# JacobMackay/beifong

Hardware: AMD Instinct MI355X
Metric: Mrays/s (closest + any-hit BVH queries), Bus.obj-class radar scene (higher is better)
Workload: dtype f32

## Files before the change

beifong_amd/csrc/bf_api.cpp:

```cpp
#include <algorithm>
#include <cmath>
#include <cstdarg>
#include <cstdio>
#include <cstring>
#include <limits>
#include <new>
#include <string>

#include <dlfcn.h>
#if defined(__has_include) && __has_include(<rccl/rccl.h>)
#include <rccl/rccl.h>
#else
extern "C" {
typedef struct ncclComm *ncclComm_t;
typedef enum { ncclSuccess = 0 } ncclResult_t;
typedef enum { ncclFloat = 7 } ncclDataType_t;
typedef enum { ncclSum = 0 } ncclRedOp_t;
ncclResult_t ncclCommInitAll(ncclComm_t *comm, int ndev, const int *devlist);
ncclResult_t ncclCommDestroy(ncclComm_t comm);
ncclResult_t ncclAllReduce(const void *sendbuff, void *recvbuff, size_t count, ncclDataType_t datatype, ncclRedOp_t op, ncclComm_t comm,
                           hipStream_t stream);
ncclResult_t ncclGroupStart(void);
ncclResult_t ncclGroupEnd(void);
const char *ncclGetErrorString(ncclResult_t result);
}
#endif

#include <map>
#include <mutex>

#include "bf_scene.h"


static thread_local std::string g_err;

bf_status fail(bf_status st, const char *fmt, ...) {
    char buf[512];
    va_list ap;
    va_start(ap, fmt);
    vsnprintf(buf, sizeof(buf), fmt, ap);
    va_end(ap);
    g_err = buf;
    return st;
}

namespace {
template <typename T> bf_status upload(const std::vector<T> &v, const T **out, std::vector<void *> &owned, uint64_t &bytes) {
    *out = nullptr;
    if (v.empty()) return BF_OK;
    void *p = nullptr;
    HIP_TRY(hipMalloc(&p, v.size() * sizeof(T)));
    owned.push_back(p);
    HIP_TRY(hipMemcpy(p, v.data(), v.size() * sizeof(T), hipMemcpyHostToDevice));
    bytes += v.size() * sizeof(T);
    *out = reinterpret_cast<const T *>(p);
    return BF_OK;
}
}

static bf_tunables read_tunables() {
    bf_tunables t;
    auto num = [](const char *name, long long dflt) -> long long {
        const char *e = getenv(name);
        return e ? strtoll(e, nullptr, 10) : dflt;
    };
    t.pool = (uint32_t) std::max<long long>(1024, std::min<long long>(num("BF_WF_POOL", 1ll << 24), 1ll << 26));
    t.tail = num("BF_WF_TAIL", -1);
    t.trace_refill = (uint32_t) num("BF_TRACE_REFILL", bfd::kTraceRefill);
    t.trace_stragglers = (uint32_t) num("BF_TRACE_STRAGGLERS", bfd::kTraceStragglers);
    t.shade_chain = (uint32_t) std::max<long long>(1, num("BF_SHADE_CHAIN", bfd::kShadeChain));
    t.row_jobs = (uint32_t) num("BF_TAIL_ROWJOBS", bfd::kTailRowJobs);
    t.shade_waves = (int) std::max<long long>(1, std::min<long long>(4, num("BF_SHADE_WAVES", 3)));
    {
        const long long w = num("BF_TRACE_WAVES", 5);
        t.trace_waves = w < 5 ? 4 : (w > 5 ? 6 : 5);
    }
    t.tail_waves = num("BF_TAIL_WAVES", 3) == 2 ? 2 : 3;
    t.tail_spread = (unsigned) std::max<long long>(1, num("BF_TAIL_SPREAD", 1));
    t.tail_blocks = (unsigned) std::max<long long>(0, num("BF_TAIL_BLOCKS", 0));
    t.tail_share = (int) num("BF_TAIL_SHARE", -1);
    t.allow_plan = num("BF_WF_SYNC", 0) == 0;
    t.roll_iters = (uint32_t) std::max<long long>(0, std::min<long long>(32, num("BF_ROLL_ITERS", 0)));
    t.roll_live = (uint32_t) std::max<long long>(0, std::min<long long>(num("BF_ROLL_LIVE", 0), 1ll << 30));
    t.no_wide = getenv("BF_NO_WIDE_BVH") != nullptr;
    t.quant = num("BF_QUANT_BVH", 0) != 0;
    t.wide_rows_log = (int) num("BF_WIDE_ROWS_LOG", -1);
    t.lean = num("BF_LEAN", 1) != 0;
    t.tab_cache = num("BF_TAB_CACHE", 1) != 0;
    t.shade_split = num("BF_SHADE_SPLIT", 0) != 0;
    t.chain_min = (uint32_t) std::max<long long>(0, std::min<long long>(num("BF_CHAIN_MIN", 16), 64));
    t.grid_share = (uint32_t) std::max<long long>(0, std::min<long long>(num("BF_GRID_SHARE", 3), 16));
    t.grid_small = (uint32_t) std::max<long long>(0, std::min<long long>(num("BF_GRID_SMALL", 1ll << 22), 1ll << 30));
    t.roll_join = num("BF_ROLL_JOIN", 1) != 0;
    t.debug_surv_batches = (uint32_t) std::max<long long>(0, std::min<long long>(num("BF_DEBUG_SURV_BATCHES", 0), 1 << 14));
    return t;
}

extern "C" {

int bf_version(void) { return BF_ABI_VERSION; }
uint32_t bf_abi_sizeof(uint32_t which) {
    static const uint32_t sizes[BF_ABI_STRUCTS] = {sizeof(bf_material), sizeof(bf_shape), sizeof(bf_emitter), sizeof(bf_sensor),
                                                   sizeof(bf_scene_desc), sizeof(bf_launch), sizeof(bf_path_record), sizeof(bf_stats),
                                                   sizeof(bf_scene_info), sizeof(bf_batch)};
    return which < BF_ABI_STRUCTS ? sizes[which] : 0u;
}
uint64_t bf_abi_fingerprint(void) { return BF_ABI_FINGERPRINT; }
const char *bf_last_error(void) { return g_err.c_str(); }

int bf_device_count(void) {
    int n = 0;
    if (hipGetDeviceCount(&n) != hipSuccess) return 0;
    return n;
}

bf_status bf_set_device(int device) {
    HIP_TRY(hipSetDevice(device));
    return BF_OK;
}

static uint32_t film_pixels(const bf_launch *lp) {
    return (lp->spp && lp->film_width && lp->film_height) ? lp->film_width * lp->film_height : 1u;
}

uint32_t bf_launch_channels(const bf_launch *lp) {
    if (!lp) return 0;
    if (lp->flags & BF_FLAG_MOMENT) {
        switch (lp->mode) {
            case BF_MODE_PATH: return 11 * film_pixels(lp);
            case BF_MODE_RANGE: return (11 + 2 * lp->bins) * film_pixels(lp);
            case BF_MODE_TIME: return (11 + 6 * lp->bins) * film_pixels(lp);
            case BF_MODE_RECEIVE_RAW: return (4 + lp->phase_bins) * lp->bins * lp->bins_y;
            case BF_MODE_RECEIVE_IQ: return 5 * lp->bins * lp->bins_y;
        }
        return 0;
    }
    switch (lp->mode) {
        case BF_MODE_PATH: return 5 * film_pixels(lp);
        case BF_MODE_RANGE: return (5 + lp->bins) * film_pixels(lp);
        case BF_MODE_TIME: return (5 + 3 * lp->bins) * film_pixels(lp);
        case BF_MODE_RECEIVE_RAW: return (3 + lp->phase_bins) * lp->bins * lp->bins_y;
        case BF_MODE_RECEIVE_IQ: return 3 * lp->bins * lp->bins_y;
    }
    return 0;
}

uint32_t bf_scene_launch_channels(const bf_scene *scene, const bf_launch *lp) {
    const uint32_t n = bf_launch_channels(lp);
    if (scene && lp && (lp->flags & BF_FLAG_AOV) && scene->run.aov.n && lp->mode <= BF_MODE_TIME && !(lp->flags & (BF_FLAG_MOMENT | BF_FLAG_CLASSES))) {
        const uint64_t all = (uint64_t) n + (uint64_t) film_pixels(lp) * (bf_aov_floats(scene->run.aov.n, scene->run.aov.types) + 4u);
        return all > UINT32_MAX ? 0u : (uint32_t) all;
    }
    if (!scene || !lp || !(lp->flags & BF_FLAG_CLASSES)) return n;
    const uint64_t all = (uint64_t) n * std::max(1u, bfd::scene_n_classes(scene->d));
    return all > UINT32_MAX ? 0u : (uint32_t) all;
}

bf_status bf_scene_destroy(bf_scene *s) {
    if (!s) return BF_OK;
    (void) s->run.last.wait();
    if (s->run.roll.open && s->peers_rolling) s->peers_rolling->fetch_sub(1, std::memory_order_relaxed);
    for (void *p : s->owned) (void) hipFree(p);
    for (auto &st : s->stage) {
        if (st.ev) {
            (void) hipEventSynchronize(st.ev);
            (void) hipEventDestroy(st.ev);
        }
        if (st.host) (void) hipHostFree(st.host);
        if (st.dev) (void) hipFree(st.dev);
    }
    delete s;
    return BF_OK;
}

bf_status stage_acquire(const bf_scene *sc, size_t bytes, bf_scene::Stage **out) {
    bf_scene::Stage &st = sc->stage[sc->stage_next];
    sc->stage_next = (sc->stage_next + 1) % bf_scene::kStageSlots;
    if (st.busy) {
        HIP_TRY(hipEventSynchronize(st.ev));
        st.busy = false;
    }
    if (st.cap < bytes) {
        if (st.host) (void) hipHostFree(st.host);
        if (st.dev) (void) hipFree(st.dev);
        st.host = st.dev = nullptr;
        st.cap = 0;
        const size_t cap = std::max<size_t>(4096, (bytes + 4095) & ~size_t(4095));
        HIP_TRY(hipHostMalloc(&st.host, cap));
        HIP_TRY(hipMalloc(&st.dev, cap));
        st.cap = cap;
    }
    if (!st.ev) HIP_TRY(hipEventCreateWithFlags(&st.ev, hipEventDisableTiming));
    *out = &st;
    return BF_OK;
}
bf_status stage_commit(bf_scene::Stage *st, size_t bytes, hipStream_t stream) {
    HIP_TRY(hipMemcpyAsync(st->dev, st->host, bytes, hipMemcpyHostToDevice, stream));
    HIP_TRY(hipEventRecord(st->ev, stream));
    st->busy = true;
    return BF_OK;
}
bf_status stage_release_after(bf_scene::Stage *st, hipStream_t stream) {
    HIP_TRY(hipEventRecord(st->ev, stream));
    st->busy = true;
    return BF_OK;
}

static_assert(bf::kTopNodes == bfd::kTopNodes, "the builder's breadth-first prefix is what wf_trace caches");
static_assert(bfd::CTR_GUARD + 2 == bfd::CTR_COUNT && bfd::CTR_SURV_GUARD + 1 == bfd::CTR_COUNT,
              "the two sticky guard words are the last counters: renders clear the ones before them");

namespace {
struct TriMeta {
    uint32_t prim, shape;
    const float *n0, *n1, *n2;
    const float *uv0, *uv1, *uv2;
};
}

static bf_status gather_triangles(const bf_scene_desc *desc, std::vector<bf::BuildTri> &btris, std::vector<TriMeta> &meta, bool &any_normals,
// ... 903 lines not shown
```

beifong_amd/csrc/bf_render.cpp:

```cpp
#include "bf_scene.h"

#include <algorithm>
#include <cmath>
#include <cstdlib>
#include <cstring>
#include <limits>
#include <vector>

namespace {
struct Kernels {
    decltype(&bfk_launch_render) render;
    decltype(&bfk_wf_shade) shade;
    decltype(&bfk_wf_trace) trace;
    decltype(&bfk_launch_tail) tail;
};
const Kernels kExact = {bfk_launch_render, bfk_wf_shade, bfk_wf_trace, bfk_launch_tail};
const Kernels kFast = {bfk_launch_render_fast, bfk_wf_shade_fast, bfk_wf_trace_fast, bfk_launch_tail_fast};
const Kernels kMoment = {bfk_launch_render_moment, bfk_wf_shade_moment, bfk_wf_trace, bfk_launch_tail_moment};
const Kernels kClass = {bfk_launch_render_class, bfk_wf_shade_class, bfk_wf_trace, bfk_launch_tail_class};
const Kernels kAov = {bfk_launch_render_aov, bfk_wf_shade_aov, bfk_wf_trace, bfk_launch_tail_aov};
const Kernels &kernels_for(uint32_t flags) {
    return (flags & BF_FLAG_FAST) ? kFast : ((flags & BF_FLAG_MOMENT) ? kMoment : ((flags & BF_FLAG_CLASSES) ? kClass : ((flags & BF_FLAG_AOV) ? kAov : kExact)));
}
}

hipError_t RenderState::Feedback::post(const uint32_t *src, uint32_t n_, Owner owner_, hipStream_t stream, const unsigned long long *guards_src) {
    if (pending) return hipSuccess;
    hipError_t e = hipMemcpyAsync(counts, src, n_ * sizeof(uint32_t), hipMemcpyDeviceToHost, stream);
    if (e == hipSuccess && guards_src)
        e = hipMemcpyAsync((void *) guards, guards_src, 2 * sizeof(unsigned long long), hipMemcpyDeviceToHost, stream);
    if (e == hipSuccess) e = hipEventRecord(event, stream);
    if (e != hipSuccess) return e;
    pending = true;
    n = n_;
    owner = owner_;
    return hipSuccess;
}
RenderState::Feedback::Landed RenderState::Feedback::take() {
    const bool ready = pending && hipEventQuery(event) == hipSuccess;
    (void) hipGetLastError();
    if (!ready) return {nullptr, 0, kNone};
    pending = false;
    return {counts, n, owner};
}
uint32_t RenderState::Feedback::first_at_most(const uint32_t *counts, uint32_t n, uint32_t threshold) {
    uint32_t k = 0;
    while (k < n && counts[k] > threshold) ++k;
    return k;
}

RenderState::~RenderState() {
    for (void *p : pool) (void) hipFree(p);
    if (host) (void) hipHostFree(host);
    if (event) (void) hipEventDestroy(event);
    if (fb.counts) (void) hipHostFree(fb.counts);
    if (fb.event) (void) hipEventDestroy(fb.event);
    if (last.done) (void) hipEventDestroy(last.done);
    for (hipEvent_t e : timing) (void) hipEventDestroy(e);
    if (counters) (void) hipFree(counters);
    if (aov.rows) (void) hipFree(aov.rows);
    for (float *q : conv.scratch)
        if (q) (void) hipFree(q);
    if (conv.ws) (void) hipFree(conv.ws);
    if (conv.ring) (void) hipHostFree(conv.ring);
    for (hipEvent_t e : conv.ev)
        if (e) (void) hipEventDestroy(e);
}

extern "C" {

static bf_status wf_ensure(const bf_scene *scene, uint32_t capacity) {
    RenderState &run = scene->run;
    bfd::WF &wf = run.wf;
    if (wf.capacity >= capacity) return BF_OK;
    for (void *p : run.pool) (void) hipFree(p);
    run.pool.clear();
    std::memset(&wf, 0, sizeof(wf));
    run.roll_ring = nullptr;
    run.roll_offsets = nullptr;
    auto alloc = [&](void **p, size_t bytes) -> hipError_t {
        hipError_t e = hipMalloc(p, bytes);
        if (e == hipSuccess) run.pool.push_back(*p);
        return e;
    };
    size_t n = capacity, nb = capacity / 64;
    HIP_TRY(alloc((void **) &wf.recA, n * 64));
    HIP_TRY(alloc((void **) &wf.recB, n * 64));
    HIP_TRY(alloc((void **) &wf.recC, n * 64));
    HIP_TRY(alloc((void **) &run.masks, 8 * nb * sizeof(unsigned long long)));
    HIP_TRY(alloc((void **) &wf.n_live, (bfd::kWfMaxIter + 2) * sizeof(uint32_t)));
    HIP_TRY(alloc((void **) &run.roll_ring, bfd::kRollRing * sizeof(bfd::DRoll)));
    HIP_TRY(alloc((void **) &run.roll_offsets, bfd::kRollRing * sizeof(float4)));
    HIP_TRY(alloc((void **) &wf.surv_cursor, 64));
    wf.counters = run.counters;
    wf.capacity = capacity;
    if (!run.host) HIP_TRY(hipHostMalloc((void **) &run.host, 64));
    if (!run.event) HIP_TRY(hipEventCreateWithFlags(&run.event, hipEventDisableTiming));
    if (!run.fb.counts) HIP_TRY(hipHostMalloc((void **) &run.fb.counts, (bfd::kWfMaxIter + 2) * sizeof(uint32_t)));
    if (!run.fb.event) HIP_TRY(hipEventCreateWithFlags(&run.fb.event, hipEventDisableTiming));
    run.fb.guards = reinterpret_cast<volatile unsigned long long *>(run.host) + 1;
    run.plan.valid = false;
    run.fb.drop();
    return BF_OK;
}

static uint32_t wf_tail_threshold(const bf_scene *scene, uint32_t n_slots) {
    if (scene->tun.tail >= 0) return (uint32_t) scene->tun.tail;
    if (n_slots >= bfd::kTailSmallPool) return 1u << 17;
    return std::max<uint32_t>(1u << 17, std::min<uint32_t>(1u << 19, n_slots / 2));
}

namespace {
struct WfCtx {
    const bf_scene *scene;
    const Kernels *k;
    const bfd::DLaunch *lp;
    float *hist;
    bf_path_record *rec;
    hipStream_t stream;
    bool count_nodes, timed;
    size_t mask_bytes, lds_shade, lds_tail;
    unsigned grid_shade, grid_trace;
    uint32_t tail_max;
    bool alone;
};

static_assert(sizeof(int) * bfd::kStackDepth * bfd::kBlock % 16 == 0, "the stacks keep the histogram 16-byte aligned");
static size_t lds_bytes(const bfd::DLaunch &lp, uint32_t tab_cache, bool stacks) {
    return (stacks ? sizeof(int) * bfd::kStackDepth * bfd::kBlock : 0u) + ((sizeof(float) * lp.lds_floats + 15) & ~size_t(15)) +
           (tab_cache ? bfd::kTabBytes : 0u);
}
static uint32_t lds_hist(uint32_t n_chan, uint32_t flags) {
    return (n_chan <= (uint32_t) bfd::kMaxLdsHist && !(flags & BF_FLAG_GLOBAL_ATOMICS)) ? 1u : 0u;
}
}

static hipError_t wf_tic(const WfCtx &c, int kind) {
    if (!c.timed) return hipSuccess;
    const bf_scene *sc = c.scene;
    while (sc->run.timing.size() < 2 * (sc->run.ev_kind.size() + 1)) {
        hipEvent_t e;
        hipError_t he = hipEventCreate(&e);
        if (he != hipSuccess) return he;
        sc->run.timing.push_back(e);
    }
    sc->run.ev_kind.push_back(kind);
    return hipEventRecord(sc->run.timing[2 * (sc->run.ev_kind.size() - 1)], c.stream);
}
static hipError_t wf_toc(const WfCtx &c) {
    if (!c.timed) return hipSuccess;
    return hipEventRecord(c.scene->run.timing[2 * (c.scene->run.ev_kind.size() - 1) + 1], c.stream);
}
static bf_status wf_collect_timing(const bf_scene *scene, hipStream_t stream) {
    scene->run.ms[0] = scene->run.ms[1] = scene->run.ms[2] = 0.f;
    scene->run.tail_launches = scene->run.shade_launches = 0;
    if (scene->run.ev_kind.empty()) return BF_OK;
    HIP_TRY(hipStreamSynchronize(stream));
    for (size_t k = 0; k < scene->run.ev_kind.size(); ++k) {
        float ms = 0.f;
        HIP_TRY(hipEventElapsedTime(&ms, scene->run.timing[2 * k], scene->run.timing[2 * k + 1]));
        scene->run.ms[scene->run.ev_kind[k]] += ms;
        if (scene->run.ev_kind[k] == 2) ++scene->run.tail_launches;
        if (scene->run.ev_kind[k] == 1) ++scene->run.shade_launches;
    }
    scene->run.ev_kind.clear();
    return BF_OK;
}

static bf_status wf_setup(const bf_scene *scene, const Kernels &k, const bfd::DLaunch &lp, uint64_t pool_paths, float *hist_dev,
                          bf_path_record *records_dev, hipStream_t stream, bool count_nodes, bool timed, WfCtx &c, bool rolling = false) {
    uint64_t want = std::min<uint64_t>(scene->tun.pool, std::max<uint64_t>(pool_paths, 64));
    uint32_t n_main = (uint32_t) ((want + 63) & ~uint64_t(63)), n_surv = 0;
    if (rolling) {
        n_main = (uint32_t) ((std::max<uint64_t>(2 * pool_paths, 128) + 63) & ~uint64_t(63));
        const uint32_t surv_min = (uint32_t) scene->n_cus * 4u * (uint32_t) std::max(2, scene->tun.shade_waves) * 64u;
        n_surv = std::max<uint32_t>(surv_min, std::min<uint32_t>(1u << 21, (n_main / 8 + 63) & ~63u));
        if (scene->tun.debug_surv_batches) n_surv = scene->tun.debug_surv_batches * 64u;
    }
    bf_status st = wf_ensure(scene, n_main + n_surv);
    if (st != BF_OK) return st;
    bfd::WF &wf = scene->run.wf;
    wf.n_main = rolling ? n_main : (uint32_t) ((std::min<uint64_t>(wf.capacity, pool_paths) + 63) & ~uint64_t(63));
    wf.n_surv = n_surv;
    wf.n_slots = wf.n_main + wf.n_surv;
    wf.trace_refill = scene->tun.trace_refill;
    wf.trace_stragglers = scene->tun.trace_stragglers;
    wf.shade_chain = scene->tun.shade_chain;
    wf.row_jobs = scene->tun.row_jobs;
    wf.iq = lp.iq;
    wf.has_render = lp.batch != 0u ? 1u : 0u;
    wf.offsets = lp.batch_offsets;
    wf.has_dop = (lp.doppler || lp.resample) ? 1u : 0u;
    wf.box_slack = lp.box_slack;
    wf.geom_stride = lp.geom_stride;
    const size_t nb = wf.n_slots / 64;
    for (int b = 0; b < 2; ++b) {
        wf.m_alive[b] = scene->run.masks + (4 * b + 0) * nb;
        wf.m_trace[b] = scene->run.masks + (4 * b + 1) * nb;
        wf.m_shadow[b] = scene->run.masks + (4 * b + 2) * nb;
        wf.m_hit[b] = scene->run.masks + (4 * b + 3) * nb;
    }
    c.scene = scene;
    c.k = &k;
    c.lp = &lp;
    c.hist = hist_dev;
    c.rec = records_dev;
    c.stream = stream;
    c.count_nodes = count_nodes;
    c.timed = timed;
    c.mask_bytes = 4 * nb * sizeof(unsigned long long);
    wf.hit_split = scene->tun.shade_split ? 1u : 0u;
    wf.chain_min = scene->tun.chain_min;
    c.lds_shade = lds_bytes(lp, scene->d.tab_cache, false);
    c.lds_tail = lds_bytes(lp, scene->d.tab_cache, true);
    c.alone = false;
    const unsigned batches_per_block = bfd::kBlock / 64;
    const unsigned max_blocks = (unsigned) ((nb + batches_per_block - 1) / batches_per_block);
    c.grid_shade = std::max(1u, std::min((unsigned) scene->n_cus * (unsigned) std::max(2, scene->tun.shade_waves), max_blocks));
    c.grid_trace = std::max(1u, std::min((unsigned) scene->n_cus * (unsigned) scene->tun.trace_waves, max_blocks));
    if (rolling && scene->tun.grid_share > 1u && wf.n_slots < scene->tun.grid_small) {
        const unsigned peers = (unsigned) std::max(1, scene->peers_rolling->load(std::memory_order_relaxed));
        const unsigned share = std::min(peers, (unsigned) scene->tun.grid_share);
        c.grid_shade = std::max(1u, c.grid_shade / share);
        c.grid_trace = std::max(1u, c.grid_trace / share);
    }
    c.tail_max = wf_tail_threshold(scene, rolling ? wf.n_main / 2 : wf.n_slots);
    wf.surv_claims_max = (wf.n_surv / 64u) / std::max(1u, c.grid_shade * batches_per_block);
    if (rolling && scene->tun.debug_surv_batches) {
        const char *e = getenv("BF_DEBUG_SURV_CLAIMS");
        wf.surv_claims_max = e ? (uint32_t) strtoul(e, nullptr, 10) : 1u << 20;
    }
    return BF_OK;
}
static bf_status wf_iteration(const WfCtx &c, uint32_t it, int first) {
    const bf_scene *scene = c.scene;
    const bfd::WF &wf = scene->run.wf;
    const int nxt = (it & 1) ^ 1;
    HIP_TRY(hipMemsetAsync(wf.m_alive[nxt], 0, c.mask_bytes, c.stream));
    if (first != 1) {
        HIP_TRY(wf_tic(c, 1));
        HIP_TRY(c.k->shade(&scene->d, c.lp, &wf, it, first == 2 ? 3 : 0, c.hist, c.rec, c.grid_shade, c.lds_shade, c.stream,
                           scene->tun.shade_waves));
        HIP_TRY(wf_toc(c));
    }
    if (first != 0) {
        HIP_TRY(wf_tic(c, 1));
        HIP_TRY(c.k->shade(&scene->d, c.lp, &wf, it, first, c.hist, c.rec, c.grid_shade, c.lds_shade, c.stream, scene->tun.shade_waves));
        HIP_TRY(wf_toc(c));
    }
    return BF_OK;
}
static bf_status wf_trace_launch(const WfCtx &c, uint32_t it) {
    HIP_TRY(wf_tic(c, 0));
    HIP_TRY(c.k->trace(&c.scene->d, &c.scene->run.wf, it, c.count_nodes ? 1 : 0, c.grid_trace, c.stream, c.scene->tun.trace_waves));
    HIP_TRY(wf_toc(c));
    return BF_OK;
}
static bf_status wf_tail_launch(const WfCtx &c, uint32_t it, uint32_t est_live) {
    const bf_scene *scene = c.scene;
    const bool alone = c.alone;
    uint32_t share = 1;
    if (!alone && scene->tun.tail_share > 1) {
        share = scene->tun.tail_share >= 4 ? 4u : 2u;
        est_live = (uint32_t) std::min<uint64_t>((uint64_t) est_live * share, 1u << 30);
    }
    if (alone) {
        const uint32_t resident = (uint32_t) scene->n_cus * 4u * 3u;
        while (share < 4u && (uint64_t) est_live * (share * 2u) / 64u <= resident) share *= 2u;
        est_live = (uint32_t) std::min<uint64_t>((uint64_t) est_live * share, 1u << 30);
    }
    scene->run.wf.tail_share = share;
    HIP_TRY(wf_tic(c, 2));
    HIP_TRY(c.k->tail(&scene->d, c.lp, &scene->run.wf, it, est_live, c.hist, c.rec, c.count_nodes ? 1 : 0, c.lds_tail, c.stream,
                      scene->tun.tail_waves, scene->tun.tail_spread, scene->tun.tail_blocks));
    HIP_TRY(wf_toc(c));
    return BF_OK;
}
bf_status guard_error(unsigned long long lost, unsigned long long refused) {
    if (lost)
        return fail(BF_ERR_DEVICE, "wf_trace's iteration guard dropped %llu rays in an earlier render of this scene: that render's "
                                   "histogram is wrong (a traversal bug; please report the scene)", lost);
    return fail(BF_ERR_DEVICE, "a launch of a rolling sequence of this scene tried to claim %llu survivor batches beyond the size of "
                               "its survivor area (the claims were refused: no path was lost, but the sizing rule of wf_setup is "
                               "violated; please report the scene and the launch)", refused);
}
bf_status report_guards(const bf_scene *scene, unsigned long long lost, unsigned long long refused, const hipStream_t *async_on) {
    unsigned long long *g = scene->run.counters + bfd::CTR_GUARD;
    if (async_on) HIP_TRY(hipMemsetAsync(g, 0, 2 * sizeof(unsigned long long), *async_on));
    else HIP_TRY(hipMemset(g, 0, 2 * sizeof(unsigned long long)));
    scene->run.fb.drop();
    return guard_error(lost, refused);
}
static bf_status check_film_count(const unsigned long long *c, uint64_t n_paths) {
    if (c[bfd::CTR_FILM] != n_paths)
        return fail(BF_ERR_DEVICE, "%llu of %llu paths were binned: paths were lost or binned twice (a scheduling bug; please report the "
                                   "scene and the launch)", (unsigned long long) c[bfd::CTR_FILM], (unsigned long long) n_paths);
    return BF_OK;
}

static bf_status drive_planned(const WfCtx &c, uint32_t &it, uint32_t n, int first_kind, uint32_t tail_live) {
    bf_status st;
    for (uint32_t j = 0; j < n; ++j, ++it) {
        if ((st = wf_iteration(c, it, j == 0 ? first_kind : 0)) != BF_OK) return st;
        if ((st = wf_trace_launch(c, it)) != BF_OK) return st;
    }
    return wf_tail_launch(c, it, std::max<uint32_t>(tail_live + tail_live / 4, 64u * bfd::kBlock));
}
static bf_status drive_sync(const WfCtx &c, uint32_t &it, uint32_t max_iters, int first_kind, uint32_t *n_live) {
    const RenderState &run = c.scene->run;
    volatile uint32_t *hq = run.host;
    bf_status st;
    for (uint32_t j = 0; j < max_iters; ++j) {
        if ((st = wf_iteration(c, it, j == 0 ? first_kind : 0)) != BF_OK) return st;
        HIP_TRY(hipMemcpyAsync((void *) &hq[0], run.wf.n_live + it, sizeof(uint32_t), hipMemcpyDeviceToHost, c.stream));
        HIP_TRY(hipEventRecord(run.event, c.stream));
        if ((st = wf_trace_launch(c, it)) != BF_OK) return st;
        HIP_TRY(hipEventSynchronize(run.event));
        ++it;
        *n_live = hq[0];
        if (*n_live <= c.tail_max) break;
    }
    return BF_OK;
}

static bf_status aov_attach(const bf_scene *scene, uint64_t slots, bfd::DLaunch &lp);
static bf_status wf_render(const bf_scene *scene, const Kernels &k, const bfd::DLaunch &lp_in, float *hist_dev, bf_path_record *records_dev,
                           hipStream_t stream, bool count_nodes, bool stats, bool aov = false) {
    using Feedback = RenderState::Feedback;
    RenderState &run = scene->run;
    WfCtx c;
    bfd::DLaunch lp = lp_in;
    bf_status st = wf_setup(scene, k, lp, lp.n_paths, hist_dev, records_dev, stream, count_nodes, stats, c);
    if (st != BF_OK) return st;
    bfd::WF &wf = run.wf;
    if (aov && (st = aov_attach(scene, wf.n_slots, lp)) != BF_OK) return st;
    HIP_TRY(hipMemsetAsync(wf.n_live, 0, (bfd::kWfMaxIter + 2) * sizeof(uint32_t), stream));
    run.ev_kind.clear();
    RenderState::Plan &plan = run.plan;
    const Feedback::Landed fb = run.fb.take();
    if (fb.owner == Feedback::kPlan) {
        if (run.fb.guards[0] || run.fb.guards[1]) return report_guards(scene, run.fb.guards[0], run.fb.guards[1], &stream);
        const uint32_t at = Feedback::first_at_most(fb.counts, fb.n, plan.tail_max);
        plan.iters = at < fb.n ? at + 1 : std::min<uint32_t>(fb.n + 2, bfd::kWfMaxIter - 1);
        plan.tail_live = fb.counts[std::min(at, fb.n - 1)];
    }
    uint32_t it = 0;
    if (scene->tun.allow_plan && plan.valid && plan.n_paths == lp.n_paths && plan.mode == lp.mode &&
        plan.max_depth == (uint32_t) lp.max_depth && plan.n_slots == wf.n_slots && plan.tail_max == c.tail_max && plan.iters > 0) {
        if ((st = drive_planned(c, it, plan.iters, 1, plan.tail_live)) != BF_OK) return st;
        HIP_TRY(run.fb.post(wf.n_live, plan.iters, Feedback::kPlan, stream, wf.counters + bfd::CTR_GUARD));
    } else {
        uint32_t n_live = 0;
        if ((st = drive_sync(c, it, bfd::kWfMaxIter, 1, &n_live)) != BF_OK) return st;
        if (n_live > c.tail_max) return fail(BF_ERR_UNSUPPORTED, "path depth exceeded the wavefront iteration limit (%u bounces)", bfd::kWfMaxIter);
        plan = {true, lp.n_paths, lp.mode, (uint32_t) lp.max_depth, wf.n_slots, c.tail_max, it, n_live};
        run.fb.drop();
        if (n_live && (st = wf_tail_launch(c, it, n_live)) != BF_OK) return st;
    }
    run.iters = run.trace_launches = it;
    if (stats) return wf_collect_timing(scene, stream);
    run.ms[0] = run.ms[1] = run.ms[2] = 0.f;
    return BF_OK;
}

static bool roll_same_shape(const bf_launch &a, const bf_launch &b) {
    return a.mode == b.mode && a.color_mode == b.color_mode && a.n_paths == b.n_paths && a.max_depth == b.max_depth &&
           a.rr_depth == b.rr_depth && a.bins == b.bins && a.bins_y == b.bins_y && a.bin_width == b.bin_width &&
           a.time_c == b.time_c && a.flags == b.flags && a.phase_bins == b.phase_bins;
}

static bf_status offsets_slack(const bf_scene *scene, const float *offsets, uint32_t n, const char *who, float *dmax, float *slack) {
    for (uint32_t k = 0; k < n; ++k)
        for (int a = 0; a < 3; ++a) {
            const float q = offsets[3 * k + a];
            if (!std::isfinite(q)) return fail(BF_ERR_INVALID, "%s: non-finite mesh offset of render %u", who, k);
            *dmax = std::max(*dmax, std::fabs(q));
        }
    *slack = 1e-6f * (scene->mesh.origin_scale_built + 2.f * *dmax);
    return BF_OK;
}

static bf_status hand_over(const bf_scene *scene, hipStream_t from, hipStream_t to) {
    HIP_TRY(hipEventRecord(scene->run.event, from));
    HIP_TRY(hipStreamWaitEvent(to, scene->run.event, 0));
    return BF_OK;
}

static bf_status wf_roll_flush(const bf_scene *scene, hipStream_t stream, bool sync_timing) {
    using Feedback = RenderState::Feedback;
    RenderState &run = scene->run;
    RenderState::Roll &r = run.roll;
    if (!r.open) return BF_OK;
    bf_status st;
    if (stream != r.stream && (st = hand_over(scene, r.stream, stream)) != BF_OK) return st;
    bfd::DLaunch &lp = r.lp;
    WfCtx c;
    if ((st = wf_setup(scene, kernels_for(r.shape.flags), lp, (uint64_t) r.per_call * lp.batch_paths, nullptr, nullptr, stream, r.count_nodes, r.timed, c, true)) != BF_OK) return st;
    c.alone = true;
    const Feedback::Landed fb = run.fb.take();
    if (fb.owner == Feedback::kRollFlush) {
        const uint32_t at = Feedback::first_at_most(fb.counts, fb.n, c.tail_max);
        r.flush_iters = at < fb.n ? at + 1 : std::min<uint32_t>(fb.n + 2, 48u);
        r.flush_live = fb.counts[std::min(at, fb.n - 1)];
    }
    if (r.it + 2u * 64u > bfd::kWfMaxIter) r.it &= 1u;
    const uint32_t it0 = r.it;
    HIP_TRY(hipMemsetAsync(run.wf.n_live + it0, 0, 64 * sizeof(uint32_t), stream));
    if (scene->tun.allow_plan && r.flush_iters > 0) {
        if ((st = drive_planned(c, r.it, r.flush_iters, 0, r.flush_live)) != BF_OK) return st;
        HIP_TRY(run.fb.post(run.wf.n_live + it0, r.it - it0, Feedback::kRollFlush, stream));
    } else {
        uint32_t n_live = 0;
        if ((st = drive_sync(c, r.it, 48u, 0, &n_live)) != BF_OK) return st;
        r.flush_iters = r.it - it0;
        r.flush_live = n_live;
        if (n_live && (st = wf_tail_launch(c, r.it, n_live)) != BF_OK) return st;
    }
    run.iters += r.it - it0;
    run.trace_launches += r.it - it0;
    r.open = false;
    scene->peers_rolling->fetch_sub(1, std::memory_order_relaxed);
    r.multi = false;
    lp.multi = 0u;
    if ((st = scene->ends.go_home(stream)) != BF_OK) return st;
    if (sync_timing) return wf_collect_timing(scene, stream);
    return BF_OK;
}

static bf_status wf_roll_render(const bf_scene *scene, const bf_launch *launch, const bf_batch *batch, const bfd::DLaunch &lp_in,
                                float *hist_dev, bf_path_record *records_dev, hipStream_t stream) {
    RenderState::Roll &r = scene->run.roll;
    bf_status st;
    const uint32_t K = batch ? batch->n_renders : 1u;
    const bool with_offsets = batch && batch->mesh_offsets && scene->d.n_tris != 0;
    if (r.open && (!roll_same_shape(r.shape, *launch) || r.per_call != K || r.offsets != with_offsets ||
                   r.count + K > bfd::kRollRing || r.stream != stream)) {
        if ((st = wf_roll_flush(scene, r.stream, false)) != BF_OK) return st;
        if (r.stream != stream && (st = hand_over(scene, r.stream, stream)) != BF_OK) return st;
    }
    const bool opening = !r.open;
    if (opening) {
        if (!roll_same_shape(r.shape, *launch) || r.per_call != K) r.iters = r.flush_iters = r.flush_live = 0;
        r.shape = *launch;
        r.lp = lp_in;
        r.lp.batch = 1u;
        r.lp.batch_paths = launch->n_paths;
        r.lp.batch_seeds = nullptr;
        r.lp.batch_offsets = nullptr;
        r.lp.box_slack = 0.f;
        r.lp.has_records = 0u;
        r.per_call = K;
        r.multi = false;
        r.offsets = with_offsets;
        r.dmax = 0.f;
        r.count = 0;
        r.it = 0;
        r.stream = stream;
        r.count_nodes = (launch->flags & BF_FLAG_STATS) != 0;
        r.timed = (launch->flags & BF_FLAG_TIMING) != 0;
        r.window = 1;
        r.lp.lds_hist = lds_hist(lp_in.n_chan, launch->flags);
        if (r.lp.lds_hist) r.window = std::max<uint32_t>(1u, std::min<uint32_t>(bfd::kRollWindow, (uint32_t) bfd::kMaxLdsHist / std::max(1u, lp_in.n_chan)));
        HIP_TRY(hipMemsetAsync(scene->run.counters, 0, sizeof(unsigned long long) * bfd::CTR_GUARD, stream));
        scene->run.ev_kind.clear();
        scene->run.iters = scene->run.trace_launches = 0;
    }
    const bool fresh_pool = opening;
    const uint32_t k = r.count, newest = k + K - 1u;
    bfd::DLaunch &lp = r.lp;
    lp.n_paths = (uint64_t) (k + K) * lp.batch_paths;
    if (r.multi) {
        lp.multi = 1u;
        lp.lean = 0u;
        scene->run.last_variant &= (uint32_t) (BF_VARIANT_FAST | BF_VARIANT_MOMENT);
    }
    lp.roll_newest = newest;
    lp.roll_lo = newest + 1u > r.window ? newest + 1u - r.window : 0u;
    lp.n_chan_all = (lp.roll_newest - lp.roll_lo + 1u) * lp.n_chan;
    lp.base_off = lp.lds_hist ? r.window * lp.n_chan : 0u;
    lp.lds_floats = lp.base_off + ((r.shape.flags & BF_FLAG_MOMENT) ? bfd::kRollBaseChMoment : bfd::kRollBaseCh) * bfd::kRollBase;
    WfCtx c;
    if (with_offsets && (st = offsets_slack(scene, batch->mesh_offsets, K, "bf_render_batch", &r.dmax, &lp.box_slack)) != BF_OK) return st;
    if ((st = wf_setup(scene, kernels_for(r.shape.flags), lp, (uint64_t) K * lp.batch_paths, nullptr, nullptr, stream, r.count_nodes, r.timed, c, true)) != BF_OK) return st;
    lp.roll = scene->run.roll_ring;
    lp.batch_offsets = with_offsets ? scene->run.roll_offsets : nullptr;
    scene->run.wf.offsets = lp.batch_offsets;
    {
        const uint32_t n_main = scene->run.wf.n_main, lo = (uint32_t) (((uint64_t) k * lp.batch_paths) % n_main);
        scene->run.wf.wake_b0 = lo / 64u;
        scene->run.wf.wake_nb = (uint32_t) std::min<uint64_t>(n_main / 64u, ((uint64_t) (lo % 64u) + (uint64_t) K * lp.batch_paths + 63u) / 64u);
    }
    if (fresh_pool) HIP_TRY(hipMemsetAsync(scene->run.wf.surv_cursor, 0, 2 * sizeof(uint32_t), stream));
    const uint32_t n_chan1 = lp.n_chan;
    if (records_dev) lp.has_records = 1u;
    for (uint32_t j = 0; j < K; ++j) {
        bfd::DRoll d;
        d.seed = (batch && batch->seeds) ? batch->seeds[j] : launch->seed;
        d.path_offset = launch->path_offset;
        d.hist = hist_dev + (size_t) j * n_chan1;
        d.records = records_dev ? records_dev + (size_t) j * lp.batch_paths : nullptr;
        d.rects = scene->d.rects;
        d.shapes = scene->d.shapes;
        d.emitters = scene->d.emitters;
        d.materials = scene->d.materials;
        d.sensor = scene->d.sensor;
        d.c = scene->d.c;
        d.lambda_min = scene->d.lambda_min;
        d.lambda_max = scene->d.lambda_max;
        d.pad = 0u;
        HIP_TRY(bfk_roll_set(scene->run.roll_ring, scene->run.roll_offsets, (k + j) & (bfd::kRollRing - 1u), &d,
                             with_offsets ? batch->mesh_offsets + 3 * j : nullptr, stream));
    }
    const RenderState::Feedback::Landed fb = scene->run.fb.take();
    if (fb.owner == RenderState::Feedback::kRollCall && !scene->tun.roll_iters) {
        const uint32_t live_max = scene->tun.roll_live ? scene->tun.roll_live : std::max<uint32_t>(3u << 19, scene->run.wf.n_main / 4u);
        r.iters = std::min<uint32_t>(RenderState::Feedback::first_at_most(fb.counts, fb.n, live_max) + 1u, 16u);
    }
    if (scene->tun.roll_iters) r.iters = scene->tun.roll_iters;
    if (r.iters == 0) r.iters = 2;
    if (r.it + 2u * 64u > bfd::kWfMaxIter) r.it &= 1u;
    const uint32_t it0 = r.it, I = r.iters;
    HIP_TRY(hipMemsetAsync(scene->run.wf.n_live + it0, 0, I * sizeof(uint32_t), stream));
    for (uint32_t j = 0; j < I; ++j) {
        const uint32_t it = r.it;
        if ((st = wf_iteration(c, it, j == 0 ? (opening ? 1 : 2) : 0)) != BF_OK) return st;
        if ((st = wf_trace_launch(c, it)) != BF_OK) return st;
        ++r.it;
    }
    scene->run.iters += I;
    scene->run.trace_launches += I;
    HIP_TRY(scene->run.fb.post(scene->run.wf.n_live + it0, I, RenderState::Feedback::kRollCall, stream));
    if (!r.open) scene->peers_rolling->fetch_add(1, std::memory_order_relaxed);
    r.open = true;
    r.count += K;
    return BF_OK;
}

void fill_stats(const bf_scene *scene, const unsigned long long *c, uint64_t n_paths, bf_stats *st) {
    std::memset(st, 0, sizeof(*st));
    st->n_paths = n_paths;
    st->n_rays_closest = c[bfd::CTR_CLOSEST];
    st->n_rays_shadow = c[bfd::CTR_SHADOW];
    st->n_nodes_visited = c[bfd::CTR_NODES];
    st->n_nodes_lds = c[bfd::CTR_NODES_LDS];
    st->n_tris_tested = c[bfd::CTR_TRIS];
    st->n_invalid = c[bfd::CTR_INVALID];
    st->n_bounces = c[bfd::CTR_BOUNCES];
    st->n_rays_tail = c[bfd::CTR_TAIL_RAYS];
    st->n_rays_traced = c[bfd::CTR_TRACED];
    st->n_nodes_tail = c[bfd::CTR_TAIL_NODES];
    st->n_wnodes_tail = c[bfd::CTR_TAIL_WNODES];
    st->n_tris_tail = c[bfd::CTR_TAIL_TRIS];
    st->n_bounces_tail = c[bfd::CTR_TAIL_BOUNCES];
    st->n_shade_loads = c[bfd::CTR_SHADE_LOADS];
    st->n_shade_stores = c[bfd::CTR_SHADE_STORES];
    st->n_shade_shadow = c[bfd::CTR_SHADE_SHADOW];
    st->n_shade_rays = c[bfd::CTR_SHADE_RAYS];
    st->n_guard = c[bfd::CTR_GUARD];
    st->trace_ms = scene->run.ms[0];
    st->shade_ms = scene->run.ms[1];
    st->tail_ms = scene->run.ms[2];
    st->n_launches_trace = scene->run.trace_launches;
    st->n_bounce_iters = scene->run.iters;
    st->n_launches_tail = scene->run.tail_launches;
    st->n_launches_shade = scene->run.shade_launches;
    st->kernel_variant = scene->run.last_variant;
}

void add_stats(bf_stats &a, const bf_stats &b) {
    a.n_paths += b.n_paths;
    a.n_rays_closest += b.n_rays_closest;
    a.n_rays_shadow += b.n_rays_shadow;
    a.n_nodes_visited += b.n_nodes_visited;
    a.n_tris_tested += b.n_tris_tested;
    a.n_invalid += b.n_invalid;
    a.n_bounces += b.n_bounces;
    a.kernel_ms += b.kernel_ms;
    a.trace_ms += b.trace_ms;
    a.shade_ms += b.shade_ms;
    a.tail_ms += b.tail_ms;
    a.n_launches_trace += b.n_launches_trace;
    a.n_bounce_iters += b.n_bounce_iters;
    a.n_rays_tail += b.n_rays_tail;
    a.n_rays_traced += b.n_rays_traced;
    a.n_nodes_lds += b.n_nodes_lds;
    a.n_nodes_tail += b.n_nodes_tail;
    a.n_wnodes_tail += b.n_wnodes_tail;
    a.n_tris_tail += b.n_tris_tail;
    a.n_bounces_tail += b.n_bounces_tail;
    a.n_shade_loads += b.n_shade_loads;
    a.n_shade_stores += b.n_shade_stores;
    a.n_shade_shadow += b.n_shade_shadow;
    a.n_shade_rays += b.n_shade_rays;
    a.n_guard += b.n_guard;
    a.kernel_variant |= b.kernel_variant;
// ... 596 lines not shown
```

beifong_amd/csrc/bf_scene.h:

```cpp
#pragma once
#include <hip/hip_runtime.h>

#include <atomic>
#include <functional>
#include <memory>
#include <vector>

#include "bf_build.h"
#include "bf_bvh.h"
#include "bf_converge.h"
#include "bf_device.h"
#include "bf_launch.h"
#include "bf_wavefront.h"

#define HIP_TRY(expr)                                                                              \
    do {                                                                                           \
        hipError_t e_ = (expr);                                                                    \
        if (e_ != hipSuccess) return fail(BF_ERR_DEVICE, "%s: %s", #expr, hipGetErrorString(e_)); \
    } while (0)

inline int32_t bfd_no_node() { return INT32_MIN; }
constexpr size_t kTriPad = 4;

struct bf_geometry {
    std::vector<void *> owned;
    struct MeshTopo {
        uint32_t n_vertices = 0, n_faces = 0, prim0 = 0;
        bool has_normals = false;
        std::vector<uint32_t> indices;
    };
    std::vector<MeshTopo> topo;
    uint4 *corners = nullptr;
    struct NormalIndex {
        uint32_t *offset = nullptr;
        uint4 *entries = nullptr;
        ~NormalIndex() {
            if (offset) (void) hipFree(offset);
            if (entries) (void) hipFree(entries);
        }
    };
    std::vector<std::shared_ptr<const NormalIndex>> normal_index;
    ~bf_geometry() {
        for (void *p : owned) (void) hipFree(p);
    }
};

struct bf_tunables {
    uint32_t pool = 1u << 24;
    int64_t tail = -1;
    uint32_t trace_refill = bfd::kTraceRefill, trace_stragglers = bfd::kTraceStragglers;
    uint32_t shade_chain = bfd::kShadeChain, row_jobs = bfd::kTailRowJobs;
    int shade_waves = 3, trace_waves = 5, tail_waves = 3;
    unsigned tail_spread = 1, tail_blocks = 0;
    int tail_share = -1;
    bool allow_plan = true;
    uint32_t roll_iters = 0;
    uint32_t roll_live = 0;
    bool no_wide = false, quant = false;
    int wide_rows_log = -1;
    bool lean = true;
    bool tab_cache = true;
    bool shade_split = false;
    uint32_t chain_min = 16;
    uint32_t grid_share = 3;
    uint32_t grid_small = 1u << 22;
    bool roll_join = true;
    uint32_t debug_surv_batches = 0;
};

struct __attribute__((visibility("hidden"))) MeshSkin {
    uint32_t n_bones = 0, n_vertices = 0;
    void *block = nullptr;
    const float4 *weight = nullptr;
    const uint4 *index = nullptr;
    const float *rest_pos = nullptr;
    const float *rest_nrm = nullptr;
    float rest_abs[3] = {0.f, 0.f, 0.f};
    double weight_sum = 0.0;
    float pivot_min = 1.f;
    std::vector<uint8_t> bone_used;
    ~MeshSkin() {
        if (block) (void) hipFree(block);
    }
};

struct __attribute__((visibility("hidden"))) MeshMorph {
    uint32_t n_targets = 0, n_vertices = 0;
    void *block = nullptr;
    const float *rest_pos = nullptr;
    const float *rest_nrm = nullptr;
    const float *dpos = nullptr;
    const float *dnrm = nullptr;
    float rest_abs[3] = {0.f, 0.f, 0.f};
    std::vector<float> delta_abs;
    ~MeshMorph() {
        if (block) (void) hipFree(block);
    }
};

struct __attribute__((visibility("hidden"))) MeshState {
    float4 *tris0 = nullptr, *nodes0 = nullptr, *wnodes0 = nullptr;
    float4 *normals0 = nullptr;
    bool geom_private = false;
    bool base_private = false;
    bool normals_private = false;
    bool normals0_private = false;
    bool normals_moved = false;
    bool deformed = false;
    int pose_kind = 0;
    std::vector<float> pose_xf;
    float origin_scale_built = 0.f;
    struct Refit {
        bool ready = false;
        bool have_boxes = false;
        std::vector<uint32_t> off4, off16;
        uint32_t *lvl4 = nullptr, *lvl16 = nullptr;
        float4 *ubox4 = nullptr, *ubox16 = nullptr;
        float *xf = nullptr;
        std::vector<float> mesh_box;
    } refit;
    float4 *arena = nullptr;
    size_t arena_cap = 0;
    uint32_t batch_versions = 0;
    size_t batch_rows = 0;
    uint32_t *bad = nullptr, *bad_host = nullptr;
    hipEvent_t bad_ev = nullptr;
    mutable bool bad_pending = false;
    mutable uint32_t bad_reported = 0;
    void *vtx_host = nullptr, *vtx_dev = nullptr;
    size_t vtx_cap = 0;
    hipEvent_t vtx_ev = nullptr;
    std::vector<std::shared_ptr<const MeshSkin>> skins;
    std::vector<std::shared_ptr<const MeshMorph>> morphs;
    float *pose_vtx = nullptr;
    size_t pose_vtx_cap = 0;
    std::vector<uint8_t> normal_mode;
    float *nrm_vtx = nullptr;
    size_t nrm_vtx_cap = 0;
    bool recomputes(uint32_t shape) const { return shape < normal_mode.size() && normal_mode[shape] == BF_NORMALS_RECOMPUTE; }
    std::vector<uint8_t> skin_mode;
    bool skins_dq(uint32_t shape) const { return shape < skin_mode.size() && skin_mode[shape] == BF_SKIN_DUAL_QUATERNION; }

    struct Base { const float4 *tris, *nodes, *wnodes, *normals; };
    Base base(const bfd::DScene &d) const {
        return {tris0 ? tris0 : d.tris, tris0 ? nodes0 : d.nodes, tris0 ? wnodes0 : d.wnodes, normals0 ? normals0 : d.normals};
    }
    struct Bytes { size_t tris, normals, nodes, wnodes; };
    static Bytes bytes(uint32_t n_tris, uint32_t n_nodes, size_t wide_nodes) {
        return {((size_t) n_tris * bfd::kTriStride + kTriPad) * sizeof(float4), (size_t) n_tris * 3 * sizeof(float4), (size_t) n_nodes * 8 * sizeof(float4),
                wide_nodes * 32 * sizeof(float4)};
    }
    static Bytes bytes(const bfd::DScene &d) { return bytes(d.n_tris, d.n_nodes, d.wnodes ? d.n_wnodes : 0); }
    bf_status own_normals(bfd::DScene &d, std::vector<void *> &owned, const char *who);
    void reset_after_rebuild(float4 *tris0_, float4 *nodes0_, float4 *wnodes0_, float4 *normals0_);
    ~MeshState();
};

struct __attribute__((visibility("hidden"))) RenderState {
    bfd::WF wf{};
    std::vector<void *> pool;
    unsigned long long *masks = nullptr;
    bfd::DRoll *roll_ring = nullptr;
    float4 *roll_offsets = nullptr;
    unsigned long long *counters = nullptr;
    uint32_t *host = nullptr;
    hipEvent_t event = nullptr;
    std::vector<hipEvent_t> timing;
    std::vector<int> ev_kind;
    float ms[3] = {0, 0, 0};
    uint32_t iters = 0, trace_launches = 0, tail_launches = 0, shade_launches = 0;
    uint32_t last_variant = 0;
    struct Aov {
        uint32_t n = 0;
        uint32_t types[BF_MAX_AOVS] = {};
        float *rows = nullptr;
        uint64_t rows_floats = 0;
    } aov;
    struct Roll {
        bool open = false;
        uint32_t count = 0;
        uint32_t it = 0;
        bf_launch shape;
        bfd::DLaunch lp;
        hipStream_t stream = nullptr;
        bool count_nodes = false, timed = false;
        uint32_t per_call = 1;
        bool offsets = false;
        float dmax = 0.f;
        uint32_t window = 1;
        uint32_t iters = 0;
        uint32_t flush_iters = 0;
        uint32_t flush_live = 0;
        bool multi = false;
    } roll;
    struct Plan {
        bool valid = false;
        uint64_t n_paths = 0;
        uint32_t mode = 0, max_depth = 0, n_slots = 0, tail_max = 0;
        uint32_t iters = 0, tail_live = 0;
    } plan;
    struct Feedback {
        enum Owner { kNone, kPlan, kRollCall, kRollFlush };
        uint32_t *counts = nullptr;
        volatile unsigned long long *guards = nullptr;
        hipEvent_t event = nullptr;
        bool pending = false;
        uint32_t n = 0;
        Owner owner = kNone;
        struct Landed {
            const uint32_t *counts;
            uint32_t n;
            Owner owner;
        };
        hipError_t post(const uint32_t *src, uint32_t n, Owner owner, hipStream_t stream, const unsigned long long *guards_src = nullptr);
        Landed take();
        void drop() { pending = false; }
        static uint32_t first_at_most(const uint32_t *counts, uint32_t n, uint32_t threshold);
    } fb;
    struct LastUse {
        hipStream_t stream = nullptr;
        hipEvent_t done = nullptr;
        bool has = false;
        hipError_t wait() const { return has ? hipEventSynchronize(done) : hipSuccess; }
    } last;
    struct Converge {
        static constexpr uint32_t kRing = 4;
        float *scratch[2] = {nullptr, nullptr};
        size_t cap = 0;
        bfd::ConvWork *ws = nullptr;
        bfd::ConvResult *ring = nullptr;
        hipEvent_t ev[2] = {nullptr, nullptr};
    } conv;
    ~RenderState();
};

struct __attribute__((visibility("hidden"))) EndpointState {
    struct Image {
        std::vector<bfd::DRect> rects;
        std::vector<bfd::DShape> shapes;
        std::vector<bfd::DEmitter> emitters;
        std::vector<bfd::DMaterial> materials;
        bfd::DSensor sensor;
        uint32_t n_tris = 0;
        uint32_t window_t = 0, window_f = 0;
        uint32_t film_w = 1, film_h = 1;
        float c = 0.f, lambda_min = 0.f, lambda_max = 0.f;
        float origin_scale = 0.f;
    };
    uint32_t n_rects = 0, n_shapes = 0, n_emitters = 0, n_materials = 0;
    std::vector<uint32_t> emitter_types;
    bool any_back_material = false;
    bool any_resample = false;
    bfd::DSensor sensor_host;
    uint32_t film_w = 1, film_h = 1;
    uint32_t adc_t = 0, adc_f = 0;
    std::vector<bfd::DShape> shapes_host;
    struct Layout {
        size_t o_rects = 0, o_shapes = 0, o_emit = 0, o_mat = 0, o_sensor = 0, total = 0;
    } lay;
    char *home = nullptr;
    size_t stride = 0;
    char *pool = nullptr;
    uint32_t next = 0;
    bool in_pool = false;
    bfd::DScene *d = nullptr;
    std::vector<float *> array_dev;
    std::vector<uint32_t> array_n;
    float *sensor_array_dev = nullptr;
    uint32_t sensor_array_n = 0;
    uint32_t *classes = nullptr;

    void apply(const Image &img, bool tab_cache);
    void pack(const Image &img, char *blk) const;
    void point_at(const char *blk);
    bf_status claim(char **blk);
    void joined() { ++next, in_pool = true; }
    bf_status go_home(hipStream_t stream);
    ~EndpointState();
};

struct bf_scene {
    bfd::DScene d;
    bf_tunables tun;
    std::shared_ptr<bf_geometry> geom;
    std::shared_ptr<char> geom_token;
    std::shared_ptr<std::atomic<int>> peers_rolling;
    mutable std::atomic_flag busy = ATOMIC_FLAG_INIT;
    std::vector<void *> owned;
    bf_scene_info info;
    int device = 0;
    int n_cus = 256;
    MeshState mesh;
    mutable RenderState run;
    mutable EndpointState ends;
    static constexpr int kStageSlots = 8;
    struct Stage {
        void *host = nullptr, *dev = nullptr;
        size_t cap = 0;
        hipEvent_t ev = nullptr;
        bool busy = false;
    };
    mutable Stage stage[kStageSlots];
    mutable int stage_next = 0;
};

#pragma GCC visibility push(hidden)
struct BusyGuard {
    const bf_scene *s;
    bool ok;
    int prev_device = -1;
    explicit BusyGuard(const bf_scene *sc) : s(sc), ok(sc && !sc->busy.test_and_set(std::memory_order_acquire)) {
        if (ok) {
            int cur = -1;
            if (hipGetDevice(&cur) == hipSuccess && cur != sc->device && hipSetDevice(sc->device) == hipSuccess) prev_device = cur;
        }
    }
    ~BusyGuard() {
        if (prev_device >= 0) (void) hipSetDevice(prev_device);
        if (ok) s->busy.clear(std::memory_order_release);
    }
};
struct DeviceGuard {
    int prev = -1;
    explicit DeviceGuard(int device) {
        int cur = -1;
        if (hipGetDevice(&cur) == hipSuccess && cur != device && hipSetDevice(device) == hipSuccess) prev = cur;
    }
    ~DeviceGuard() {
        if (prev >= 0) (void) hipSetDevice(prev);
    }
};
#define BF_ENTER_AS(scene, name)                                                                                          \
    BusyGuard busy_guard_(scene);                                                                                         \
    if (!busy_guard_.ok)                                                                                                  \
        return fail(BF_ERR_INVALID, "%s: the scene handle is in use by another host thread (one call at a time per handle; " \
                                    "bf_scene_clone gives every thread / stream its own)", name)
#define BF_ENTER(scene) BF_ENTER_AS(scene, __func__)

extern "C" {
bf_status fail(bf_status st, const char *fmt, ...);
bf_status stage_acquire(const bf_scene *sc, size_t bytes, bf_scene::Stage **out);
bf_status stage_commit(bf_scene::Stage *st, size_t bytes, hipStream_t stream);
bf_status stage_release_after(bf_scene::Stage *st, hipStream_t stream);
// ... 38 lines not shown
```

beifong_amd/csrc/bf_wavefront.h:

```cpp
#pragma once
#include <hip/hip_runtime.h>

#include "bf_ns.h"
#include <stddef.h>
#include <stdint.h>

BF_NS_BEGIN

constexpr uint32_t kWfMaxIter = 4096;
constexpr uint32_t kShadeChain = 8;
constexpr uint32_t kTraceRefill = 32;
constexpr uint32_t kTraceStragglers = 12;
constexpr uint32_t kTraceBlocksPerCU = 8;
constexpr uint32_t kTailSmallPool = 1u << 22;
constexpr uint32_t kTailRowJobs = 12;

#define BF_HD __host__ __device__ __forceinline__

struct WF {
    float4 *recA, *recB, *recC;
    BF_HD float4 &ray0(uint32_t i) const { return recA[4 * (size_t) i + 0]; }
    BF_HD float4 &ray1(uint32_t i) const { return recA[4 * (size_t) i + 1]; }
    BF_HD float4 &hit(uint32_t i) const { return recA[4 * (size_t) i + 2]; }
    BF_HD uint32_t &hit_prim(uint32_t i) const { return reinterpret_cast<uint32_t *>(recA + 4 * (size_t) i + 3)[0]; }
    BF_HD uint32_t &render(uint32_t i) const { return reinterpret_cast<uint32_t *>(recA + 4 * (size_t) i + 3)[1]; }
    BF_HD float &dop(uint32_t i) const { return reinterpret_cast<float *>(recA + 4 * (size_t) i + 3)[2]; }
    BF_HD uint32_t &cls(uint32_t i) const { return reinterpret_cast<uint32_t *>(recA + 4 * (size_t) i + 3)[3]; }
    BF_HD float4 &sa(uint32_t i) const { return recB[4 * (size_t) i + 0]; }
    BF_HD float4 &sb(uint32_t i) const { return recB[4 * (size_t) i + 1]; }
    BF_HD uint4 &sd(uint32_t i) const { return reinterpret_cast<uint4 *>(recB)[4 * (size_t) i + 2]; }
    BF_HD float4 &se(uint32_t i) const { return recB[4 * (size_t) i + 3]; }
    BF_HD float4 &sh0(uint32_t i) const { return recC[4 * (size_t) i + 0]; }
    BF_HD float4 &sh1(uint32_t i) const { return recC[4 * (size_t) i + 1]; }
    BF_HD float &sh2(uint32_t i) const { return reinterpret_cast<float *>(recC + 4 * (size_t) i + 2)[0]; }
    BF_HD float &sh3(uint32_t i) const { return reinterpret_cast<float *>(recC + 4 * (size_t) i + 2)[1]; }
    BF_HD uint32_t &occ(uint32_t i) const { return reinterpret_cast<uint32_t *>(recC + 4 * (size_t) i + 2)[2]; }
    BF_HD float4 &sh23(uint32_t i) const { return recC[4 * (size_t) i + 2]; }
    uint32_t has_render;
    uint32_t has_dop;
    const float4 *offsets;
    float box_slack;
    uint32_t geom_stride;
    unsigned long long *m_alive[2];
    unsigned long long *m_trace[2];
    unsigned long long *m_shadow[2];
    unsigned long long *m_hit[2];
    uint32_t hit_split;
    uint32_t chain_min;
    uint32_t reserved[3];
    uint32_t *n_live;
    unsigned long long *counters;
    uint32_t trace_refill, trace_stragglers;
    uint32_t iq;
    uint32_t shade_chain;
    uint32_t row_jobs;
    uint32_t n_slots;
    uint32_t capacity;
    uint32_t n_main, n_surv;
    uint32_t *surv_cursor;
    uint32_t wake_b0, wake_nb;
    uint32_t tail_share;
    uint32_t surv_claims_max;
};
static_assert(sizeof(WF) == 216 && offsetof(WF, n_live) == 136, "WF is a kernel argument: its layout is the kernels' argument layout");

BF_NS_END
```

Before: 1708.

## Rework rolling flush planning and cap tail blocks to resident occupancy

```diff
diff --git a/beifong_amd/csrc/bf_api.cpp b/beifong_amd/csrc/bf_api.cpp
--- a/beifong_amd/csrc/bf_api.cpp
+++ b/beifong_amd/csrc/bf_api.cpp
@@ -66,6 +66,7 @@
     };
     t.pool = (uint32_t) std::max<long long>(1024, std::min<long long>(num("BF_WF_POOL", 1ll << 24), 1ll << 26));
     t.tail = num("BF_WF_TAIL", -1);
+    t.tail_flush = num("BF_WF_TAIL_FLUSH", -1);
     t.trace_refill = (uint32_t) num("BF_TRACE_REFILL", bfd::kTraceRefill);
     t.trace_stragglers = (uint32_t) num("BF_TRACE_STRAGGLERS", bfd::kTraceStragglers);
     t.shade_chain = (uint32_t) std::max<long long>(1, num("BF_SHADE_CHAIN", bfd::kShadeChain));
diff --git a/beifong_amd/csrc/bf_render.cpp b/beifong_amd/csrc/bf_render.cpp
--- a/beifong_amd/csrc/bf_render.cpp
+++ b/beifong_amd/csrc/bf_render.cpp
@@ -104,8 +104,9 @@
     return BF_OK;
 }
 
-static uint32_t wf_tail_threshold(const bf_scene *scene, uint32_t n_slots) {
+static uint32_t wf_tail_threshold(const bf_scene *scene, uint32_t n_slots, bool alone = false) {
     if (scene->tun.tail >= 0) return (uint32_t) scene->tun.tail;
+    if (alone && scene->tun.tail_flush >= 0) return (uint32_t) std::min<int64_t>(scene->tun.tail_flush, 0xffffffffll);
     if (n_slots >= bfd::kTailSmallPool) return 1u << 17;
     return std::max<uint32_t>(1u << 17, std::min<uint32_t>(1u << 19, n_slots / 2));
 }
@@ -264,15 +265,21 @@
         share = scene->tun.tail_share >= 4 ? 4u : 2u;
         est_live = (uint32_t) std::min<uint64_t>((uint64_t) est_live * share, 1u << 30);
     }
+    unsigned block_cap = scene->tun.tail_blocks;
     if (alone) {
         const uint32_t resident = (uint32_t) scene->n_cus * 4u * 3u;
         while (share < 4u && (uint64_t) est_live * (share * 2u) / 64u <= resident) share *= 2u;
         est_live = (uint32_t) std::min<uint64_t>((uint64_t) est_live * share, 1u << 30);
+        const unsigned per_cu = std::max<unsigned>(1u, std::min<unsigned>((unsigned) scene->tun.tail_waves, (unsigned) (bfd::kLdsPerCU / std::max<size_t>(c.lds_tail, 1))));
+        if (!block_cap && scene->run.wf.n_main / 2u >= bfd::kTailSmallPool) {
+            block_cap = (unsigned) scene->n_cus * per_cu;
+            est_live = std::max<uint32_t>(est_live, block_cap * (uint32_t) bfd::kBlock);
+        }
     }
     scene->run.wf.tail_share = share;
     HIP_TRY(wf_tic(c, 2));
     HIP_TRY(c.k->tail(&scene->d, c.lp, &scene->run.wf, it, est_live, c.hist, c.rec, c.count_nodes ? 1 : 0, c.lds_tail, c.stream,
-                      scene->tun.tail_waves, scene->tun.tail_spread, scene->tun.tail_blocks));
+                      scene->tun.tail_waves, scene->tun.tail_spread, block_cap));
     HIP_TRY(wf_toc(c));
     return BF_OK;
 }
@@ -397,21 +404,31 @@
     WfCtx c;
     if ((st = wf_setup(scene, kernels_for(r.shape.flags), lp, (uint64_t) r.per_call * lp.batch_paths, nullptr, nullptr, stream, r.count_nodes, r.timed, c, true)) != BF_OK) return st;
     c.alone = true;
+    c.tail_max = wf_tail_threshold(scene, run.wf.n_main / 2, true);
+    const uint32_t min_iters = scene->tun.tail_flush >= 0 && scene->tun.tail < 0 ? 0u : 1u;
     const Feedback::Landed fb = run.fb.take();
-    if (fb.owner == Feedback::kRollFlush) {
+    if (r.flush_planned && r.flush_tail_max != c.tail_max) r.flush_planned = false;
+    if (fb.owner == Feedback::kRollFlush && r.flush_planned && fb.n > 0) {
         const uint32_t at = Feedback::first_at_most(fb.counts, fb.n, c.tail_max);
-        r.flush_iters = at < fb.n ? at + 1 : std::min<uint32_t>(fb.n + 2, 48u);
-        r.flush_live = fb.counts[std::min(at, fb.n - 1)];
-    }
+        r.flush_iters = std::max<uint32_t>(min_iters, at < fb.n ? at : std::min<uint32_t>(fb.n + 1, 48u));
+        r.flush_live = fb.counts[std::min<uint32_t>(std::max(at, min_iters), fb.n - 1)];
+    }
+    const uint32_t prev = r.it - 1u;
     if (r.it + 2u * 64u > bfd::kWfMaxIter) r.it &= 1u;
     const uint32_t it0 = r.it;
     HIP_TRY(hipMemsetAsync(run.wf.n_live + it0, 0, 64 * sizeof(uint32_t), stream));
-    if (scene->tun.allow_plan && r.flush_iters > 0) {
+    if (scene->tun.allow_plan && r.flush_planned) {
         if ((st = drive_planned(c, r.it, r.flush_iters, 0, r.flush_live)) != BF_OK) return st;
-        HIP_TRY(run.fb.post(run.wf.n_live + it0, r.it - it0, Feedback::kRollFlush, stream));
+        if (it0 == prev + 1u) HIP_TRY(run.fb.post(run.wf.n_live + prev, 1u + r.it - it0, Feedback::kRollFlush, stream));
     } else {
-        uint32_t n_live = 0;
-        if ((st = drive_sync(c, r.it, 48u, 0, &n_live)) != BF_OK) return st;
+        volatile uint32_t *hq = run.host;
+        HIP_TRY(hipMemcpyAsync((void *) &hq[0], run.wf.n_live + prev, sizeof(uint32_t), hipMemcpyDeviceToHost, stream));
+        HIP_TRY(hipEventRecord(run.event, stream));
+        HIP_TRY(hipEventSynchronize(run.event));
+        uint32_t n_live = hq[0];
+        if ((n_live > c.tail_max || min_iters) && (st = drive_sync(c, r.it, 48u, 0, &n_live)) != BF_OK) return st;
+        r.flush_planned = true;
+        r.flush_tail_max = c.tail_max;
         r.flush_iters = r.it - it0;
         r.flush_live = n_live;
         if (n_live && (st = wf_tail_launch(c, r.it, n_live)) != BF_OK) return st;
@@ -440,7 +457,7 @@
     }
     const bool opening = !r.open;
     if (opening) {
-        if (!roll_same_shape(r.shape, *launch) || r.per_call != K) r.iters = r.flush_iters = r.flush_live = 0;
+        if (!roll_same_shape(r.shape, *launch) || r.per_call != K) r.iters = r.flush_iters = r.flush_live = 0, r.flush_planned = false;
         r.shape = *launch;
         r.lp = lp_in;
         r.lp.batch = 1u;
diff --git a/beifong_amd/csrc/bf_scene.h b/beifong_amd/csrc/bf_scene.h
--- a/beifong_amd/csrc/bf_scene.h
+++ b/beifong_amd/csrc/bf_scene.h
@@ -48,6 +48,7 @@
 struct bf_tunables {
     uint32_t pool = 1u << 24;
     int64_t tail = -1;
+    int64_t tail_flush = -1;
     uint32_t trace_refill = bfd::kTraceRefill, trace_stragglers = bfd::kTraceStragglers;
     uint32_t shade_chain = bfd::kShadeChain, row_jobs = bfd::kTailRowJobs;
     int shade_waves = 3, trace_waves = 5, tail_waves = 3;
@@ -189,6 +190,8 @@
         float dmax = 0.f;
         uint32_t window = 1;
         uint32_t iters = 0;
+        bool flush_planned = false;
+        uint32_t flush_tail_max = 0;
         uint32_t flush_iters = 0;
         uint32_t flush_live = 0;
         bool multi = false;
diff --git a/beifong_amd/csrc/bf_wavefront.h b/beifong_amd/csrc/bf_wavefront.h
--- a/beifong_amd/csrc/bf_wavefront.h
+++ b/beifong_amd/csrc/bf_wavefront.h
@@ -12,6 +12,7 @@
 constexpr uint32_t kTraceRefill = 32;
 constexpr uint32_t kTraceStragglers = 12;
 constexpr uint32_t kTraceBlocksPerCU = 8;
+constexpr size_t kLdsPerCU = 160u << 10;
 constexpr uint32_t kTailSmallPool = 1u << 22;
 constexpr uint32_t kTailRowJobs = 12;
 
```

Result: no change. 1716 (median of 5 runs) (+0.5%).
